# psaegert/bcnf

Measured on AMD Instinct MI355X. Metric: NLL-training samples/sec + log_prob max-abs-err vs ref, trajectory_FC_small, higher is better.
Workload: dtype f32; 1 GPU; trajectory_FC_small NLL training step (configs[1]); batch_per_gpu=4096, global_batch=4096, parallelism=dp1, hip_graph=True, n_blocks=32, n_conditions=80

## Files before the change

### bcnf_amd/csrc/bcnf_device.h

```cpp
#pragma once
#include <hip/hip_runtime.h>
#include <stdint.h>

#include <atomic>
#include <mutex>
#include <utility>

#include "../../include/bcnf_amd.h"

#define BCNF_WG 256
#define BCNF_ROWS 16
#define BCNF_TSTRIDE 17

typedef float floatx4 __attribute__((ext_vector_type(4)));

namespace bcnf_rt {
inline int hip_status(hipError_t e) { return e == hipSuccess ? 0 : BCNF_ERR_HIP_BASE + (int)e; }

constexpr size_t LDS_MAX = 160 * 1024;

struct Lds {
  size_t bytes, request;
  Lds(size_t b) : bytes(b), request(b) {}
  Lds(size_t b, size_t ceiling) : bytes(b), request(ceiling > b ? ceiling : b) {}
};

template <auto Kernel, typename... Args>
int launch(dim3 grid, dim3 block, Lds lds, hipStream_t stream, Args&&... args) {
  if (lds.bytes > LDS_MAX) return BCNF_ERR_UNSUPPORTED;
  if (lds.bytes > 0) {
    static std::atomic<size_t> granted{0};
    static std::mutex grow;
    if (lds.request > granted.load(std::memory_order_acquire)) {
      std::lock_guard<std::mutex> lk(grow);
      if (lds.request > granted.load(std::memory_order_relaxed)) {
        const hipError_t e = hipFuncSetAttribute(reinterpret_cast<const void*>(Kernel),
                                                 hipFuncAttributeMaxDynamicSharedMemorySize, (int)lds.request);
        if (e != hipSuccess) return hip_status(e);
        granted.store(lds.request, std::memory_order_release);
      }
    }
  }
  Kernel<<<grid, block, lds.bytes, stream>>>(std::forward<Args>(args)...);
  return hip_status(hipGetLastError());
}
}

constexpr int BCNF_GU = 8;
__device__ __forceinline__ void gather2_rows(const int64_t* __restrict__ idx, int n, int rpw,
                                             const float* __restrict__ s0, int c0, float* __restrict__ d0,
                                             const float* __restrict__ s1, int c1, float* __restrict__ d1,
                                             const long long* __restrict__ cursor, int bx) {
  if (cursor) idx += cursor[0] * n;
  const int r0 = bx * rpw, r1 = r0 + rpw < n ? r0 + rpw : n;
  const int cw = c0 + c1, total = (r1 - r0) * cw;
  for (int e0 = 0; e0 < total; e0 += BCNF_GU * BCNF_WG) {
    int r[BCNF_GU], col[BCNF_GU];
    long long src[BCNF_GU];
    float v[BCNF_GU];
#pragma unroll
    for (int u = 0; u < BCNF_GU; ++u) {
      int e = e0 + u * BCNF_WG + threadIdx.x;
      e = e < total ? e : total - 1;
      const int rr = e / cw;
      r[u] = r0 + rr;
      col[u] = e - rr * cw;
      src[u] = idx[r[u]];
    }
#pragma unroll
    for (int u = 0; u < BCNF_GU; ++u)
      v[u] = col[u] < c0 ? s0[src[u] * c0 + col[u]] : s1[src[u] * c1 + (col[u] - c0)];
#pragma unroll
    for (int u = 0; u < BCNF_GU; ++u) {
      if (e0 + u * BCNF_WG + (int)threadIdx.x >= total) continue;
      if (col[u] < c0)
        d0[r[u] * c0 + col[u]] = v[u];
      else
        d1[r[u] * c1 + (col[u] - c0)] = v[u];
    }
  }
}

struct BcnfGatherArgs {
  const int64_t* idx;
  const long long* cursor;
  const float* s0;
  float* d0;
  const float* s1;
  float* d1;
  int n, rpw, c0, c1, nwg;
};

inline void gather2_plan(long long n, int* rpw, int* nwg) {
  const int w = n < 512 ? (int)n : 512;
  *rpw = w > 0 ? (int)((n + w - 1) / w) : 1;
  *nwg = w > 0 ? (int)((n + *rpw - 1) / *rpw) : 0;
}
// ... 326 lines not shown
```

### bcnf_amd/csrc/bcnf_stack_bwd.hip

```cpp
#include "bcnf_stack_internal.h"
#include "bcnf_stack_rec.h"

namespace {
using namespace bcnf_small;
using bcnf_rt::launch;

#if BCNF_STAMPS
__device__ unsigned long long g_phase[32];
#endif

template <int NH>
struct BwdJobs {
  static constexpr int ND = NH + 6, NA = NH + 1;
  static constexpr int NW = NH + 2, NS = NH + 6;
  static constexpr int SUM_OFF = NW * 256;
  static constexpr int BLK = NW * 256 + NS * 16;
  __device__ static constexpr int wb(int c) { return c < NH ? c : NH; }
};

template <int NH>
__device__ __forceinline__ void bwd_grad_jobs(const float* __restrict__ Td, const float* __restrict__ Ta,
                                              float* __restrict__ out, int hw) {
  using J = BwdJobs<NH>;
  const int l64 = threadIdx.x & 63, q = l64 >> 4, r = l64 & 15;
  constexpr int UW = (J::NW + 3) / 4, US = (J::NS + 3) / 4;
  floatx4 a[UW], bv[UW], v[US];
  const int o = 4 * tile_slot(r, q);
#pragma unroll
  for (int u = 0; u < UW; ++u) {
    const int c = hw + 4 * u < J::NW ? hw + 4 * u : J::NW - 1;
    a[u] = *reinterpret_cast<const floatx4*>(Td + c * TILE + o);
    bv[u] = *reinterpret_cast<const floatx4*>(Ta + J::wb(c) * TILE + o);
  }
#pragma unroll
  for (int u = 0; u < US; ++u) {
    const int c = hw + 4 * u < J::NS ? hw + 4 * u : J::NS - 1;
    v[u] = *reinterpret_cast<const floatx4*>(Td + c * TILE + o);
  }
  floatx4 acc[UW];
#pragma unroll
  for (int u = 0; u < UW; ++u) acc[u] = floatx4{0.f, 0.f, 0.f, 0.f};
#pragma unroll
  for (int t = 0; t < 4; ++t)
#pragma unroll
    for (int u = 0; u < UW; ++u) acc[u] = mfma4(a[u][t], bv[u][t], acc[u]);
#pragma unroll
  for (int u = 0; u < US; ++u) {
    const float tot = sum_rows4((v[u][0] + v[u][1]) + (v[u][2] + v[u][3]));
    if (hw + 4 * u < J::NS && q == 0) out[J::SUM_OFF + 16 * (hw + 4 * u) + r] = tot;
  }
#pragma unroll
  for (int u = 0; u < UW; ++u)
    if (hw + 4 * u < J::NW) st4_wt_mfma(reinterpret_cast<floatx4*>(out + 256 * (hw + 4 * u)) + l64, acc[u]);
}

constexpr int BWD_WG = 2 * BCNF_WG;
constexpr int BWD_G4 = 3;

template <int NH>
__global__ __launch_bounds__(BWD_WG) void k_backward(BcnfLayout L, const float* __restrict__ pk,
                                                     const float* __restrict__ dz, const float* __restrict__ dldj,
                                                     const float* __restrict__ dloss, int nll, long long B,
                                                     const float* __restrict__ arec,
                                                     float* __restrict__ dy, float* __restrict__ d1,
                                                     float* __restrict__ slab_all, long long slab_stride,
                                                     const float* __restrict__ nll_part, float* __restrict__ loss_out,
                                                     uint64_t* rng_w, int32_t* guard) {
  static_assert(NH + 3 <= 4 * BWD_G4, "derivative slot");
  extern __shared__ __attribute__((aligned(16))) float smem[];
  using AR = ActRec<NH>;
  using RBk = RecB<NH>;
  using J = BwdJobs<NH>;
  const int RBL = 16 * L.RB;
  float* recB = smem;
  float* dT = recB + 2 * RING;
  float* aT = dT + 2 * J::ND * TILE;
  floatx4* gsl = reinterpret_cast<floatx4*>(aT + 3 * J::NA * TILE);
  const int nb = L.nb;
  const float* pbk = pk + L.pb_off;
  const bool helper = threadIdx.x >= BCNF_WG;
  const int t8 = (int)threadIdx.x & (BCNF_WG - 1);
  const int j = t8 & 15, s = sample_of(t8);
  const int tix = tile_ix(s, j);
  unsigned long long ph_t = BCNF_STAMPS ? __builtin_amdgcn_s_memtime() : 0ULL, ph_acc[4] = {0, 0, 0, 0};
#define PHS(i)                                                                                   \
  if (BCNF_STAMPS) {                                                                             \
    const unsigned long long _t = __builtin_amdgcn_s_memtime();                                  \
    ph_acc[i] += _t - ph_t;                                                                      \
    ph_t = _t;                                                                                   \
  }

  if (helper) {
    const int hw = __builtin_amdgcn_readfirstlane(t8 >> 6);
    float* slab = slab_all + (long long)blockIdx.x * slab_stride;
    const floatx4* arl = reinterpret_cast<const floatx4*>(arec) + (long long)blockIdx.x * AR::AR4 * BCNF_WG + t8;
    const long long ars = (long long)gridDim.x * AR::AR4 * BCNF_WG;
    struct Prep {
      Stage<STAGE_REC> sr;
      floatx4 rec[AR::AR4];
      float rec1[AR::AR1 > 0 ? AR::AR1 : 1];
      float sa, ba;
    };
    const float* ar1l = arec + ar1_off(nb, gridDim.x, AR::AR4) + (long long)blockIdx.x * AR::AR1 * BCNF_WG + t8;
    const long long ar1s = (long long)gridDim.x * AR::AR1 * BCNF_WG;
    auto prep_load = [&](Prep& P, int k) {
      P.sr.load_t(pbk + (long long)k * RBL, RBL, t8);
#pragma unroll
      for (int i = 0; i < AR::AR4; ++i) P.rec[i] = arl[(long long)k * ars + i * BCNF_WG];
#pragma unroll
      for (int i = 0; i < AR::AR1; ++i) P.rec1[i] = ar1l[(long long)k * ar1s + i * BCNF_WG];
      const float* an = pbk + (long long)k * RBL + j * L.RB + RBk::AN;
      P.sa = an[0];
      P.ba = an[1];
    };
    auto prep_store = [&](Prep& P, int k) {
#pragma unroll
      for (int i = 0; i < AR::AR4; ++i) asm volatile("" : "+v"(P.rec[i]));
#pragma unroll
      for (int i = 0; i < AR::AR1; ++i) asm volatile("" : "+v"(P.rec1[i]));
      asm volatile("" : "+v"(P.sa), "+v"(P.ba));
      float ar[4 * AR::AR4 + AR::AR1];
#pragma unroll
      for (int i = 0; i < AR::AR4; ++i) {
        ar[4 * i] = P.rec[i][0];
        ar[4 * i + 1] = P.rec[i][1];
        ar[4 * i + 2] = P.rec[i][2];
        ar[4 * i + 3] = P.rec[i][3];
      }
#pragma unroll
      for (int i = 0; i < AR::AR1; ++i) ar[4 * AR::AR4 + i] = P.rec1[i];
      float* ta = aT + (k % 3) * J::NA * TILE + tix;
#pragma unroll
      for (int l = 1; l <= NH; ++l) ta[l * TILE] = ar[AR::act(l - 1)];
      ta[0] = fmaf(P.sa, ar[AR::YA], P.ba);
      float gs[4 * BWD_G4];
#pragma unroll
      for (int l = 0; l < NH; ++l) gs[l] = ar[AR::gd(l)];
      gs[NH] = ar[AR::S];
      gs[NH + 1] = ar[AR::YA];
      gs[NH + 2] = ar[AR::YB];
#pragma unroll
      for (int i = NH + 3; i < 4 * BWD_G4; ++i) gs[i] = 0.f;
      floatx4* gd = gsl + (k & 1) * BWD_G4 * BCNF_WG + t8;
#pragma unroll
      for (int i = 0; i < BWD_G4; ++i) gd[i * BCNF_WG] = floatx4{gs[4 * i], gs[4 * i + 1], gs[4 * i + 2], gs[4 * i + 3]};
      P.sr.store_t(recB + (k & 1) * RING, t8);
    };
    Prep Pa, Pb;
    prep_load(Pa, nb - 1);
    prep_load(Pb, nb >= 2 ? nb - 2 : 0);
    prep_store(Pa, nb - 1);
    __syncthreads();
    auto step = [&](int k, Prep& Pc, Prep& Pnext) {
      PHS(0)
      prep_load(Pnext, k >= 2 ? k - 2 : 0);
      PHS(1)
      if (k + 1 < nb)
        bwd_grad_jobs<NH>(dT + ((k + 1) & 1) * J::ND * TILE, aT + ((k + 1) % 3) * J::NA * TILE,
                          slab + (long long)(k + 1) * J::BLK, hw);
      PHS(2)
      if (k >= 1) prep_store(Pc, k - 1);
      PHS(3)
      __syncthreads();
    };
    for (int k = nb - 1; k >= 0; k -= 2) {
      step(k, Pb, Pa);
      if (k == 0) break;
      step(k - 1, Pa, Pb);
    }
    bwd_grad_jobs<NH>(dT, aT, slab, hw);
  } else {
    const int tid = t8;
    const long long b = (long long)blockIdx.x * 16 + s;
    const bool valid = b < B;
    const long long bc = valid ? b : B - 1;
    const int D = L.D, Da = L.Da, Db = L.Db;
    float* d1l = d1 + bc * 16 + j;
    float* d1_dummy = d1 + (long long)nb * B * 16 + j;
    const long long hps = B * 16;

    float gya = 0.f, gyb = 0.f, dl = 0.f;
    if (valid) {
      if (nll) {
        const float sc = (dloss ? dloss[0] + dloss[1] : 1.f) / (float)B;
        gya = (j < Da) ? dz[b * D + j] * sc : 0.f;
        gyb = (j < Db) ? dz[b * D + Da + j] * sc : 0.f;
        dl = -sc;
      } else {
        if (dz) {
          gya = (j < Da) ? dz[b * D + j] : 0.f;
          gyb = (j < Db) ? dz[b * D + Da + j] : 0.f;
        }
        if (dldj) dl = dldj[b];
      }
    }
    __syncthreads();
    PHS(0)
    for (int k = nb - 1; k >= 0; --k) {
      const int cur = k & 1;
      float gs[4 * BWD_G4];
      {
        const floatx4* gd4 = gsl + cur * BWD_G4 * BCNF_WG + tid;
#pragma unroll
        for (int i = 0; i < BWD_G4; ++i) {
          const floatx4 v = gd4[i * BCNF_WG];
          gs[4 * i] = v[0];
          gs[4 * i + 1] = v[1];
          gs[4 * i + 2] = v[2];
          gs[4 * i + 3] = v[3];
        }
      }
      float* Tt = dT + cur * J::ND * TILE + tix;
      const float* R = recB + cur * RING + j * L.RB;
      float rb[RBk::USED];
      ld_rec<0, RBk::HID>(rb, R);
      __builtin_amdgcn_sched_barrier(0);
      const float* gd = gs;
      const float S = gs[NH], ya = gs[NH + 1], yb = gs[NH + 2];
      const float an_sa = rb[RBk::AN], an_sb = rb[RBk::AN + 2], an_bb = rb[RBk::AN + 3];
      const float xb = fmaf(an_sb, yb, an_bb);
      const float e = exp_fast(S);
      float gza, gzb;
      if (QBC_DEV(L, QBC_MIX)) mix_bc(rb + RBk::QT, gya, gyb, gza, gzb);
      else mix(rb + RBk::QT, gya, gyb, gza, gzb);
      ld16(rb + RBk::HID, R + RBk::HID);
      __builtin_amdgcn_sched_barrier(0);
      const float dT_ = gzb;
      const float dS = (j < Db) ? fmaf(gzb * e, xb, dl) : 0.f;
      const float dSp = dS * (1.f - S * S);
      const float dxb = gzb * e;
      Tt[NH * TILE] = dT_;
      Tt[(NH + 1) * TILE] = dSp;
      float da = 0.f, da2 = 0.f;
      if (QBC_DEV(L, QBC_HEAD)) bc9x2(dT_, rb + RBk::TT, da, dSp, rb + RBk::ST, da2);
      else rot16x2(dT_, rb + RBk::TT, da, dSp, rb + RBk::ST, da2);
      da += da2;
#pragma unroll
      for (int l = NH; l >= 2; --l) {
        ld16(rb + RBk::HID + 16 * (NH - l + 1), R + RBk::HID + 16 * (NH - l + 1));
        __builtin_amdgcn_sched_barrier(0);
        const float dpre = da * gd[l - 1];
        Tt[(l - 1) * TILE] = dpre;
        da = rot16(dpre, rb + RBk::HID + 16 * (NH - l), 0.f);
      }
      const float dpre1 = da * gd[0];
      Tt[0] = dpre1;
      *(valid ? d1l + k * hps : d1_dummy) = dpre1;
      const float dxa = rot16(dpre1, rb + RBk::W1T, gza);
      {
        const float inv_a = (j < Da) ? __builtin_amdgcn_rcpf(an_sa) : 0.f;
        const float inv_b = (j < Db) ? __builtin_amdgcn_rcpf(an_sb) : 0.f;
        Tt[(NH + 2) * TILE] = fmaf(dxa, ya, dl * inv_a);
        Tt[(NH + 3) * TILE] = dxa;
        Tt[(NH + 4) * TILE] = fmaf(dxb, yb, dl * inv_b);
        Tt[(NH + 5) * TILE] = dxb;
      }
      gya = an_sa * dxa;
      gyb = an_sb * dxb;
      PHS(1)
      __syncthreads();
      PHS(2)
    }
    if (dy && valid) {
      if (j < Da) dy[b * D + j] = gya;
      if (j < Db) dy[b * D + Da + j] = gyb;
    }
  }
#if BCNF_STAMPS
  if (blockIdx.x == 0 && (threadIdx.x == 0 || threadIdx.x == BCNF_WG))
    for (int i = 0; i < 4; ++i) g_phase[(helper ? 4 : 0) + i] = ph_acc[i];
#endif
#undef PHS
  if (loss_out && blockIdx.x == 0) {
    __syncthreads();
    nll_finalize<BWD_WG>(nll_part, (int)gridDim.x, B, loss_out, rng_w, guard, dT);
  }
}

}

namespace bcnf_small {

int launch_backward(const BcnfLayout& L, const float* pk, const float* dz, const float* dldj, const float* dloss,
                    int nll, long long B, const float* arec, float* dy, float* d1, float* slab, const float* part,
                    float* loss_out, uint64_t* rng_w, int32_t* guard, hipStream_t st) {
  return dispatch_nh(L.NH, [&](auto nh) -> int {
    constexpr int NH = decltype(nh)::value;
    if (!layout_matches<NH>(L)) return BCNF_ERR_ARG;
    const dim3 grid((unsigned)((B + 15) / 16));
    return launch<k_backward<NH>>(grid, dim3(BWD_WG), bwd_lds_bytes(L), st, L, pk, dz, dldj, dloss, nll, B, arec, dy,
                                  d1, slab, slab_stride_of(L), part, loss_out, rng_w, guard);
  });
}

#if BCNF_STAMPS
int bwd_debug_phases(unsigned long long* out) {
  return bcnf_rt::hip_status(hipMemcpyFromSymbol(out, HIP_SYMBOL(g_phase), sizeof(g_phase)));
}
#endif

}
```

### bcnf_amd/csrc/bcnf_stack_fwd.hip

```cpp
#include "bcnf_stack_internal.h"
#include "bcnf_stack_rec.h"

namespace {
using namespace bcnf_small;
using bcnf_rt::launch;

#if BCNF_STAMPS
__device__ unsigned long long g_phase[32];
#endif

struct ProjArgs {
  const float* h;
  const float* w1c;
  const float* b1c;
  long long ldh;
  int C, Cp, NKp;
};
struct RawArgs : RawForward {};
constexpr int RAW_WQ = 8;
constexpr int RAW_SIDE_Q = 4;
__host__ __device__ constexpr int raw_hs_pitch(int C) { return 16 * ((C + 15) / 16) + 4; }
__device__ __forceinline__ long long raw_row(const RawArgs& R, long long B, long long b) {
  return R.idx ? (long long)R.idx[(R.cursor ? R.cursor[0] * B : 0) + b] : b;
}

constexpr int HP_SMAX = 16;
constexpr int FWD_SLOTS = 3;
constexpr int FWD_HP = FWD_SLOTS * 4 * 256;
constexpr int FWD_HEAD = 24;

template <int NH, bool DROP, bool SAVE, bool RAW = false>
__global__ __launch_bounds__(2 * BCNF_WG) void k_forward(BcnfLayout L, const float* __restrict__ pk,
                                                    const float* __restrict__ y, ProjArgs P,
                                                    long long B, float* __restrict__ z, float* __restrict__ ldj_out,
                                                    float* __restrict__ logp, const uint64_t* rng,
                                                    float* __restrict__ arec, float* __restrict__ nll_part,
                                                    RawArgs R) {
  extern __shared__ __attribute__((aligned(16))) float smem[];
  const int RFL = 16 * L.RF;
  float* rec = smem;
  float* hpb = rec + FWD_SLOTS * RING;
  floatx4* mkb = reinterpret_cast<floatx4*>(hpb + FWD_HP);
  float* lps = hpb + FWD_HP + FWD_SLOTS * 8 * 256;
  float* hs = lps + 4;
  using AR = ActRec<NH>;
  static_assert(NH <= 8, "two float4 of dropout multipliers");
  const int nb = L.nb;
  const float* pf = pk + L.pf_off;
  const bool helper = threadIdx.x >= BCNF_WG;
  const int t8 = (int)threadIdx.x & (BCNF_WG - 1);
  const int j = t8 & 15, s = sample_of(t8);
  const long long b = (long long)blockIdx.x * 16 + s;
  const long long bc = b < B ? b : B - 1;
  uint64_t seed = 0, off = 0;
  if (DROP) { seed = rng[0]; off = rng[1]; }
  unsigned long long ph_t = BCNF_STAMPS ? __builtin_amdgcn_s_memtime() : 0ULL, ph_acc[3] = {0, 0, 0};
  const unsigned long long ph_t0 = ph_t;
  const unsigned long long ph_r0 = BCNF_STAMPS ? __builtin_amdgcn_s_memrealtime() : 0ULL;
  unsigned long long ph_b[2] = {0, 0};
#define PHB(i)                                                 \
  if (BCNF_STAMPS) ph_b[i] = __builtin_amdgcn_s_memtime() - ph_t0;
  unsigned long long ph_p[4] = {0, 0, 0, 0};
#define PHP(i)                                                                           \
  if (BCNF_STAMPS) {                                                                     \
    asm volatile("s_waitcnt vmcnt(0) lgkmcnt(0)" ::: "memory");                          \
    ph_p[i] = __builtin_amdgcn_s_memtime() - ph_t0;                                      \
  }
#define PHF(i)                                                                                   \
  if (BCNF_STAMPS) {                                                                             \
    const unsigned long long _t = __builtin_amdgcn_s_memtime();                                  \
    ph_acc[i] += _t - ph_t;                                                                      \
    ph_t = _t;                                                                                   \
  }

  if (helper) {
    const int hw = __builtin_amdgcn_readfirstlane(t8 >> 6);
    const int l64 = t8 & 63, lr = l64 & 15, lq = l64 >> 4;
    if constexpr (RAW) {
      const int Da = L.Da, C = L.C, X = R.X, H1 = L.H[1], D = L.D, an = L.an_size;
      const int nt = (C + 15) >> 4;
      const long long row = (long long)blockIdx.x * 16 + lr;
      const float* xrow = R.xpool + raw_row(R, B, row < B ? row : B - 1) * R.ldx;
      uint32_t tw[RAW_NSP];
#pragma unroll
      for (int i = 0; i < RAW_NSP / 4; ++i) {
        const uint4 v = reinterpret_cast<const uint4*>(R.table + t8 * RAW_NSP)[i];
        tw[4 * i] = v.x;
        tw[4 * i + 1] = v.y;
        tw[4 * i + 2] = v.z;
        tw[4 * i + 3] = v.w;
      }
      const int rb16 = 16 * L.RB, ch = (rb16 + BCNF_WG - 1) / BCNF_WG, n_units = nb * ch + L.NKp;
      const uint32_t* tpb = R.table + RAW_NSP * BCNF_WG;
      uint32_t pbe[RAW_SIDE_Q];
#pragma unroll
      for (int q = 0; q < RAW_SIDE_Q; ++q) {
        const int u = blockIdx.x + q * gridDim.x, n = (u % ch) * BCNF_WG + t8;
        pbe[q] = tpb[n < rb16 ? n : 0];
      }
      asm volatile("" ::: "memory");
      uint32_t srcb[RAW_NP + RAW_NQ], dstb[RAW_NP + RAW_NQ];
#pragma unroll
      for (int i = 0; i < RAW_NP + RAW_NQ; ++i) {
        srcb[i] = (tw[i] >> 12) * 4u;
        dstb[i] = (tw[i] & 4095u) * 4u;
      }
      uint32_t zw[RAW_NZ];
#pragma unroll
      for (int i = 0; i < RAW_NZ; ++i) zw[i] = tw[RAW_NP + RAW_NQ + i] & 4095u;
      PHP(0)
      int wo[RAW_TPW];
      uint32_t wok = 0;
#pragma unroll
      for (int i = 0; i < RAW_TPW; ++i) {
// ... 269 lines not shown
        for (int u = 0; u < RAW_WQ; ++u) {
          const int i = tid + u * BCNF_WG, c = i / XQ, q = i - c * XQ;
          if (i < nq) {
            floatx4 o;
#pragma unroll
            for (int r = 0; r < 4; ++r) o[r] = 4 * q + r < X ? __uint_as_float(v[u][r]) : 0.f;
            *reinterpret_cast<floatx4*>(ws + c * RAW_KP + 4 * q) = o;
          }
        }
        for (int i = nq > RAW_WQ * BCNF_WG ? tid + RAW_WQ * BCNF_WG : nq; i < nq; i += BCNF_WG) {
          const int c = i / XQ, q = i - c * XQ;
          const auto w = __builtin_amdgcn_raw_buffer_load_b128(rW, (c * X + 4 * q) * 4, 0, 0);
          floatx4 o;
#pragma unroll
          for (int r = 0; r < 4; ++r) o[r] = 4 * q + r < X ? __uint_as_float(w[r]) : 0.f;
          *reinterpret_cast<floatx4*>(ws + c * RAW_KP + 4 * q) = o;
        }
#pragma unroll
        for (int u = 0; u < NXQ; ++u) {
          const int i = tid + u * BCNF_WG;
          if (i < 16 * (RAW_KP / 4)) {
            const int rr = i / (RAW_KP / 4), q = i - rr * (RAW_KP / 4);
            *reinterpret_cast<floatx4*>(xs + rr * RAW_KP + 4 * q) = xo[u];
            const long long bb = (long long)blockIdx.x * 16 + rr;
            if (R.xdst && bb < B && 4 * q < X) {
              float* xd = R.xdst + bb * R.ldx + 4 * q;
              if (4 * q + 3 < X) {
                __builtin_memcpy(xd, &xo[u], sizeof(floatx4));
              } else {
#pragma unroll
                for (int r = 0; r < 4; ++r)
                  if (4 * q + r < X) xd[r] = xo[u][r];
              }
            }
          }
        }
      }
      PHP(0)
      __syncthreads();
      floatx4 acc[RAW_TPW][2];
#pragma unroll
      for (int i = 0; i < RAW_TPW; ++i) acc[i][0] = acc[i][1] = floatx4{0.f, 0.f, 0.f, 0.f};
#pragma unroll
      for (int u = 0; u < RAW_KP / 16; ++u) {
        if (16 * u >= X) break;
        const floatx4 xv = *reinterpret_cast<const floatx4*>(xs + lr * RAW_KP + 16 * u + 4 * lq);
#pragma unroll
        for (int i = 0; i < RAW_TPW; ++i) {
          const int ct = cw + 4 * i;
          if (16 * ct < C) {
            const int c = 16 * ct + lr;
            const floatx4 wv = *reinterpret_cast<const floatx4*>(ws + (c < C ? c : 0) * RAW_KP + 16 * u + 4 * lq);
#pragma unroll
            for (int r = 0; r < 4; ++r) acc[i][r & 1] = mfma4(wv[r], xv[r], acc[i][r & 1]);
          }
        }
      }
#pragma unroll
      for (int i = 0; i < RAW_TPW; ++i) {
        const int ct = cw + 4 * i;
        if (16 * ct < C) {
          floatx4 o;
#pragma unroll
          for (int r = 0; r < 4; ++r) {
            const int cc = 16 * ct + 4 * lq + r;
            o[r] = cc < C ? (acc[i][0][r] + acc[i][1][r]) + (R.bf ? hb[i][r] : 0.f) : 0.f;
          }
          *reinterpret_cast<floatx4*>(hs + lr * raw_hs_pitch(C) + 16 * ct + 4 * lq) = o;
        }
      }
      PHB(0)
      __syncthreads();
      PHB(1)
      if (R.ydst && b < B) {
        if (j < Da) R.ydst[b * D + j] = ya;
        if (j < Db) R.ydst[b * D + Da + j] = yb;
      }
    } else {
      ya = (j < Da) ? y[bc * D + j] : 0.f;
      yb = (j < Db) ? y[bc * D + Da + j] : 0.f;
      ldc = pk[L.ldc_off];
    }
    __syncthreads();
    float hd[FWD_HEAD], hq4[4];
    floatx4 mk0 = {1.f, 1.f, 1.f, 1.f}, mk1 = {1.f, 1.f, 1.f, 1.f};
    auto fetch_head = [&](int sl) {
      ld_rec<0, FWD_HEAD>(hd, rec + sl * RING + j * L.RF);
      const float* hq = hpb + sl * 1024 + 16 * s + j;
#pragma unroll
      for (int i = 0; i < 4; ++i) hq4[i] = hq[256 * i];
      if (DROP) {
        mk0 = mkb[(2 * sl) * BCNF_WG + tid];
        mk1 = mkb[(2 * sl + 1) * BCNF_WG + tid];
      }
    };
    fetch_head(0);
    float ldj = 0.f;
    int cur = 0;
    int gdim = gridDim.x;
    asm volatile("" : "+s"(gdim));
    floatx4* d4 = reinterpret_cast<floatx4*>(arec) + (long long)blockIdx.x * AR::AR4 * BCNF_WG + tid;
    float* d1p = arec + ar1_off(nb, gdim, AR::AR4) + (long long)blockIdx.x * AR::AR1 * BCNF_WG + tid;
    const long long d4s = (long long)gdim * AR::AR4 * BCNF_WG, d1s = (long long)gdim * AR::AR1 * BCNF_WG;
    for (int k = 0; k < nb; ++k) {
      const int nxt = cur == FWD_SLOTS - 1 ? 0 : cur + 1;
      float rr[RecF<NH>::USED];
#pragma unroll
      for (int i = 0; i < FWD_HEAD; ++i) rr[i] = hd[i];
      const float hpk = ((hq4[0] + hq4[1]) + hq4[2]) + hq4[3];
      const float msk[8] = {mk0[0], mk0[1], mk0[2], mk0[3], mk1[0], mk1[1], mk1[2], mk1[3]};
      const float xa = fmaf(rr[0], ya, rr[1]);
      const float xb = fmaf(rr[2], yb, rr[3]);
      float T, Sp;
      float ar[AR::AR];
      ar[AR::YA] = ya;
      ar[AR::YB] = yb;
      auto emit = [&](int q) {
        if (SAVE) st4_wt(d4 + q * BCNF_WG, floatx4{ar[4 * q], ar[4 * q + 1], ar[4 * q + 2], ar[4 * q + 3]});
      };
      mlp_forward_s<NH, SAVE, DROP>(rr, rec + cur * RING + j * L.RF, xa, hpk, msk, T, Sp, ar, emit, QBC_DEV(L, QBC_W1));
      const float Sv = tanh_bf(Sp);
      const float zb = fmaf(exp_fast(Sv), xb, T);
      ldj += Sv;
      if (SAVE) {
        ar[AR::S] = Sv;
#pragma unroll
        for (int q = 0; q < AR::AR4; ++q)
          if (AR::ready_layer(q) == NH + 1) emit(q);
#pragma unroll
        for (int i = 0; i < AR::AR1; ++i) st1_wt(d1p + i * BCNF_WG, ar[4 * AR::AR4 + i]);
        d4 += d4s;
        d1p += d1s;
      }
      fetch_head(nxt);
      if (QBC_DEV(L, QBC_MIX)) mix_bc(rr + RecF<NH>::Q, xa, zb, ya, yb);
      else mix(rr + RecF<NH>::Q, xa, zb, ya, yb);
      cur = nxt;
      PHF(1)
      asm volatile("s_barrier" ::: "memory");
      PHF(2)
    }
    if constexpr (RAW) ldc = ((lps[0] + lps[1]) + lps[2]) + lps[3];
    const float ltot = row_sum16(ldj) + ldc;
    const float q2 = row_sum16(ya * ya + yb * yb);
    if (j < Da) z[bc * D + j] = ya;
    if (j < Db) z[bc * D + Da + j] = yb;
    if (j == 0 && ldj_out) ldj_out[bc] = ltot;
    if (logp && j == 0) logp[bc] = -(0.5f * q2 - ltot) - 0.5f * (float)D * 1.8378770664093454836f;
    if (nll_part && j == 0) rec[s] = (b < B) ? 0.5f * q2 - ltot : 0.f;
  }
#if BCNF_STAMPS
  if (SAVE && blockIdx.x == 0 && (threadIdx.x == 0 || threadIdx.x == BCNF_WG))
  {
    for (int i = 0; i < 3; ++i) g_phase[8 + (helper ? 4 : 0) + i] = ph_acc[i];
    g_phase[helper ? 15 : 11] = (ph_b[1] << 32) | (ph_b[0] & 0xffffffffULL);
    for (int i = 0; i < 4; ++i) g_phase[16 + (helper ? 4 : 0) + i] = ph_p[i];
    g_phase[24 + (helper ? 2 : 0)] = __builtin_amdgcn_s_memtime() - ph_t0;
    g_phase[25 + (helper ? 2 : 0)] = __builtin_amdgcn_s_memrealtime() - ph_r0;
  }
#endif
#undef PHF
#undef PHB
#undef PHP
  if (nll_part) {
    __syncthreads();
    if (threadIdx.x == 0) {
      float acc = 0.f;
      for (int i = 0; i < 16; ++i) acc += rec[i];
      nll_part[blockIdx.x] = acc;
    }
  }
}

__global__ __launch_bounds__(BCNF_WG) void k_nll_finalize(const float* __restrict__ part, int nparts, long long B,
                                                          float* __restrict__ loss_out, uint64_t* rng_w,
                                                          int32_t* guard) {
  __shared__ float red[BCNF_WG];
  nll_finalize(part, nparts, B, loss_out, rng_w, guard, red);
}

}

namespace bcnf_small {

int launch_forward(const BcnfLayout& L, const float* pk, const float* y, const float* h, const float* fold, int X,
                   int ldx, long long B, float* z, float* ldj, float* logp, bool drop, const uint64_t* rng,
                   float* arec, float* part, const RawForward* raw, hipStream_t st) {
  const BcnfLayout Lp = fold ? fold_layout(L, X, ldx) : L;
  const float* pbase = fold ? fold : pk;
  const ProjArgs P{h, pbase + Lp.w1c_off, pbase + Lp.b1c_off, (long long)Lp.ldh, Lp.C, Lp.Cp, Lp.NKp};
  const dim3 grid((unsigned)((B + 15) / 16));
  const size_t lds = fwd2_lds_bytes(L, raw != nullptr);
  const bool save = arec != nullptr;
  const RawArgs R = raw ? RawArgs{*raw} : RawArgs{};
  return dispatch_nh(L.NH, [&](auto nh) -> int {
    constexpr int NH = decltype(nh)::value;
    if (!layout_matches<NH>(L)) return BCNF_ERR_ARG;
    if (P.Cp % 16 != 0 || P.Cp / 16 > HP_SMAX || P.C > P.Cp) return BCNF_ERR_UNSUPPORTED;
#define FWD(DR, SV, RW) \
  launch<k_forward<NH, DR, SV, RW>>(grid, dim3(2 * BCNF_WG), lds, st, L, pk, y, P, B, z, ldj, logp, rng, arec, part, R)
    if (raw) return !save ? BCNF_ERR_ARG : drop ? FWD(true, true, true) : FWD(false, true, true);
    if (save) return drop ? FWD(true, true, false) : FWD(false, true, false);
    return drop ? FWD(true, false, false) : FWD(false, false, false);
#undef FWD
  });
}

int launch_nll_finalize(const float* part, int nparts, long long B, float* loss_out, uint64_t* rng_w, int32_t* guard,
                        hipStream_t st) {
  return launch<k_nll_finalize>(dim3(1), dim3(BCNF_WG), 0, st, part, nparts, B, loss_out, rng_w, guard);
}

#if BCNF_STAMPS
int fwd_debug_phases(unsigned long long* out) {
  return bcnf_rt::hip_status(hipMemcpyFromSymbol(out, HIP_SYMBOL(g_phase), sizeof(g_phase)));
}
#endif

}
```

### bcnf_amd/csrc/bcnf_stack_rec.h

```cpp
#pragma once
#include "bcnf_stack_layout.h"

#ifdef BCNF_PHASE_STAMPS
#define BCNF_STAMPS 1
#else
#define BCNF_STAMPS 0
#endif
#define QBC_DEV(L, bit) (((L).qbc & (bit)) != 0)

#pragma GCC visibility push(hidden)
namespace bcnf_small {

template <int N>
struct Stage {
  floatx4 r[N];
  __device__ __forceinline__ void load(const float* __restrict__ g, int n) { load_t(g, n, (int)threadIdx.x); }
  __device__ __forceinline__ void store(float* __restrict__ s) const { store_t(s, (int)threadIdx.x); }
  __device__ __forceinline__ void load_t(const float* __restrict__ g, int n, int t) {
    const floatx4* g4 = reinterpret_cast<const floatx4*>(g);
    const int n4 = n >> 2;
#pragma unroll
    for (int i = 0; i < N; ++i) {
      const int idx = t + i * BCNF_WG;
      r[i] = g4[idx < n4 ? idx : 0];
    }
  }
  __device__ __forceinline__ void store_t(float* __restrict__ s, int t) const {
    floatx4* s4 = reinterpret_cast<floatx4*>(s);
#pragma unroll
    for (int i = 0; i < N; ++i) s4[t + i * BCNF_WG] = r[i];
  }
};

template <bool VEC>
__device__ __forceinline__ void load_rows64(const float* __restrict__ M, long long nrows, int ncols, long long ld,
                                            long long r0, int c0, floatx4* reg, int ones = -1) {
#pragma unroll
  for (int e = 0; e < 8; ++e) {
    const int i4 = threadIdx.x + 256 * e, row = i4 >> 5, col = c0 + (i4 & 31) * 4;
    const long long r = r0 + row < nrows ? r0 + row : nrows - 1;
    if (VEC) {
      const floatx4 v = *reinterpret_cast<const floatx4*>(M + r * ld + (col < ncols ? col : 0));
#pragma unroll
      for (int q = 0; q < 4; ++q) reg[e][q] = (r0 + row < nrows && col + q < ncols) ? v[q] : 0.f;
    } else {
#pragma unroll
      for (int q = 0; q < 4; ++q) {
        const int cq = col + q;
        const float v = M[r * ld + (cq < ncols ? cq : ncols - 1)];
        reg[e][q] = (r0 + row < nrows && cq < ncols) ? v : 0.f;
      }
    }
    if (ones >= 0) {
#pragma unroll
      for (int q = 0; q < 4; ++q)
        if (col + q == ones && r0 + row < nrows) reg[e][q] = 1.f;
    }
  }
}

template <int NH>
struct RecF {
  static constexpr int B1 = 4, W1 = 8, HID = 24, T = 24 + 17 * (NH - 1), S = T + 17;
  static constexpr int Q = (S + 17 + 3) & ~3, MLP_END = (S + 17 + 3) & ~3, USED = Q + 64;
};
template <int NH>
struct RecB {
  static constexpr int AN = 0, QT = 4, TT = 68, ST = 84, HID = 100, W1T = 100 + 16 * (NH - 1);
  static constexpr int USED = W1T + 16;
};
template <int NH>
struct ActRec {
  static constexpr int YA = 2 * NH, YB = 2 * NH + 1, S = 2 * NH + 2;
  static constexpr int AR = 2 * NH + 3, AR4 = AR / 4, AR1 = AR - 4 * AR4;
  __host__ __device__ static constexpr int act(int l) { return 2 * l; }
  __host__ __device__ static constexpr int gd(int l) { return 2 * l + 1; }
  __host__ __device__ static constexpr int ready_layer(int q) {
    int r = 0;
    for (int i = 4 * q; i < 4 * q + 4; ++i) {
      const int li = i < 2 * NH ? i / 2 + 1 : (i == S ? NH + 1 : 0);
      r = li > r ? li : r;
    }
    return r;
  }
};

template <int LO, int HI>
__device__ __forceinline__ void ld_rec(float* __restrict__ rr, const float* __restrict__ R) {
  static_assert(LO % 4 == 0 && HI % 4 == 0, "record slices are 16-B aligned");
  const floatx4* R4 = reinterpret_cast<const floatx4*>(R + LO);
#pragma unroll
  for (int i = 0; i < (HI - LO) / 4; ++i) {
    const floatx4 v = R4[i];
    rr[LO + 4 * i + 0] = v.x;
    rr[LO + 4 * i + 1] = v.y;
    rr[LO + 4 * i + 2] = v.z;
    rr[LO + 4 * i + 3] = v.w;
  }
}

template <int NH>
__device__ __forceinline__ void mlp_forward(const BcnfLayout& L, const float* __restrict__ rr, float x, float hp,
                                            uint32_t bits, float& T, float& Sp) {
  using F = RecF<NH>;
  float a = x;
#pragma unroll
  for (int l = 1; l <= NH; ++l) {
    const float* w = (l == 1) ? rr + F::W1 : rr + F::HID + 17 * (l - 2);
    const float bias = (l == 1) ? hp : w[16];
    const float pre = (l == 1 && QBC_DEV(L, QBC_W1)) ? bc10(a, w, bias) : rot16(a, w, bias);
    const float m = ((bits >> (l - 1)) & 1u) ? L.keep_scale : 0.f;
    a = gelu_f(pre) * m;
  }
  T = rr[F::T + 16];
  Sp = rr[F::S + 16];
  rot16x2(a, rr + F::T, T, a, rr + F::S, Sp);
}

constexpr int FWD_AHEAD = 2;
template <int NH>
__host__ __device__ constexpr int rf_stage_end(int l) {
  return l <= NH ? 24 + 17 * (l - 1) : (l == NH + 1 ? RecF<NH>::S + 17 : RecF<NH>::USED);
}
template <int NH>
__host__ __device__ constexpr int rf_stage_q(int l) {
  int q = 6;
  for (int i = 1; i <= l; ++i) {
    const int want = (rf_stage_end<NH>(i + FWD_AHEAD < NH + 2 ? i + FWD_AHEAD : NH + 2) + 3) / 4;
    q = i >= NH + 2 ? want : (want < q + 8 ? want : q + 8);
  }
  return q;
}
template <int NH>
__device__ __forceinline__ void rf_issue(float* __restrict__ rr, const float* __restrict__ R, int l) {
  const floatx4* R4 = reinterpret_cast<const floatx4*>(R);
#pragma unroll
  for (int q = rf_stage_q<NH>(l - 1); q < rf_stage_q<NH>(l); ++q) {
    const floatx4 v = R4[q];
    rr[4 * q] = v.x;
    rr[4 * q + 1] = v.y;
    rr[4 * q + 2] = v.z;
    rr[4 * q + 3] = v.w;
  }
  __builtin_amdgcn_sched_barrier(0);
}
template <int NH, bool KEEP, bool DROP, typename Emit>
__device__ __forceinline__ void mlp_forward_s(float* __restrict__ rr, const float* __restrict__ R, float x, float hp,
                                              const float* __restrict__ msk, float& T, float& Sp, float* ar,
                                              Emit&& emit, bool qbc) {
  static_assert(RecF<NH>::HID == 24, "stage 1 reads only the prefetched head (FWD_HEAD = 24)");
  using F = RecF<NH>;
  using AR = ActRec<NH>;
  float a = x;
#pragma unroll
  for (int l = 1; l <= NH; ++l) {
    rf_issue<NH>(rr, R, l);
    const float* w = (l == 1) ? rr + F::W1 : rr + F::HID + 17 * (l - 2);
    const float pre = (l == 1 && qbc) ? bc10(a, w, hp) : rot16(a, w, (l == 1) ? hp : w[16]);
    if (KEEP) {
      float g, dg;
      gelu_fg(pre, g, dg);
      a = DROP ? g * msk[l - 1] : g;
      ar[AR::act(l - 1)] = a;
      ar[AR::gd(l - 1)] = DROP ? dg * msk[l - 1] : dg;
#pragma unroll
      for (int q = 0; q < AR::AR4; ++q)
        if (AR::ready_layer(q) == l) emit(q);
    } else if (DROP) {
      float g, dg;
      gelu_fg(pre, g, dg);
      a = g * msk[l - 1];
    } else {
      a = gelu_f(pre);
    }
  }
  rf_issue<NH>(rr, R, NH + 1);
  T = rr[F::T + 16];
  Sp = rr[F::S + 16];
  rot16x2(a, rr + F::T, T, a, rr + F::S, Sp);
  rf_issue<NH>(rr, R, NH + 2);
}

__device__ __forceinline__ void mix(const float* __restrict__ rq, float a, float b, float& na, float& nbv) {
  na = 0.f;
  nbv = 0.f;
  rot16x2(a, rq, na, a, rq + 32, nbv);
  rot16x2(b, rq + 16, na, b, rq + 48, nbv);
}

template <int NTH = BCNF_WG>
static __device__ void nll_finalize(const float* __restrict__ part, int nparts, long long B, float* __restrict__ loss_out,
                             uint64_t* rng_w, int32_t* guard, float* __restrict__ red) {
  float acc = 0.f;
  for (int i = threadIdx.x; i < nparts; i += NTH) acc += part[i];
  red[threadIdx.x] = acc;
  __syncthreads();
  for (int w = NTH / 2; w > 0; w >>= 1) {
    if ((int)threadIdx.x < w) red[threadIdx.x] += red[threadIdx.x + w];
    __syncthreads();
  }
  if (threadIdx.x == 0) {
    const float nll = red[0] / (float)B;
    loss_out[0] = nll;
    loss_out[1] = nll;
    loss_out[2] = 0.f;
    bool halt = false;
    if (guard) {
      if (guard[BCNF_GUARD_DIVERGED]) {
        guard[BCNF_GUARD_HALTED] = 1;
        halt = true;
      } else if (guard[BCNF_GUARD_CHECK] && (nll > 1e5f || isnan(nll))) {
        guard[BCNF_GUARD_DIVERGED] = 1;
      }
    }
    if (rng_w && !halt) rng_w[1] += 1;
  }
}

__device__ __forceinline__ float sum_rows4(float v) {
  const auto p = __builtin_amdgcn_permlane32_swap(__float_as_uint(v), __float_as_uint(v), false, false);
  v = __uint_as_float(p[0]) + __uint_as_float(p[1]);
  const auto p2 = __builtin_amdgcn_permlane16_swap(__float_as_uint(v), __float_as_uint(v), false, false);
  return __uint_as_float(p2[0]) + __uint_as_float(p2[1]);
}

template <int NH>
constexpr int inv_m_rf() { return round_rec(RecF<NH>::USED); }
template <int NH>
bool layout_matches(const BcnfLayout& L) {
  return L.rf_b1 == RecF<NH>::B1 && L.rf_w1 == RecF<NH>::W1 && L.rf_hid == RecF<NH>::HID && L.rf_t == RecF<NH>::T &&
         L.rf_s == RecF<NH>::S && L.rf_q == RecF<NH>::Q && L.RF == inv_m_rf<NH>() &&
         L.PMB == (NH + 6) * 256 + (NH - 1) * 16 + 96 && L.rb_w1t == RecB<NH>::W1T &&
         L.rb_hid == RecB<NH>::HID && L.rb_tt == RecB<NH>::TT && L.rb_st == RecB<NH>::ST && L.rb_qt == RecB<NH>::QT &&
         L.rb_an == RecB<NH>::AN && L.RB >= RecB<NH>::USED;
}

}
#pragma GCC visibility pop
```

Measured before the change: 31.96 million samples/s.

## Specialize kernels on compressed-record layout and load only live record words

Makes the compressed (BC) record mode a compile-time template parameter of the forward and backward kernels, replacing runtime QBC flag checks. When BC is on, the forward kernel stops loading the dead tails of the head and mixing records. The backward kernel's helper waves stage only the live quads into LDS through a precomputed index map, so fewer global loads and LDS stores are issued per block. The cost is twice as many kernel instantiations. The layout check now rejects partial QBC flag combinations.

```diff
diff --git a/bcnf_amd/csrc/bcnf_device.h b/bcnf_amd/csrc/bcnf_device.h
--- a/bcnf_amd/csrc/bcnf_device.h
+++ b/bcnf_amd/csrc/bcnf_device.h
@@ -13,6 +13,7 @@
 #define BCNF_TSTRIDE 17
 
 typedef float floatx4 __attribute__((ext_vector_type(4)));
+typedef float floatx2 __attribute__((ext_vector_type(2)));
 
 namespace bcnf_rt {
 inline int hip_status(hipError_t e) { return e == hipSuccess ? 0 : BCNF_ERR_HIP_BASE + (int)e; }
diff --git a/bcnf_amd/csrc/bcnf_stack_bwd.hip b/bcnf_amd/csrc/bcnf_stack_bwd.hip
--- a/bcnf_amd/csrc/bcnf_stack_bwd.hip
+++ b/bcnf_amd/csrc/bcnf_stack_bwd.hip
@@ -57,7 +57,7 @@
 constexpr int BWD_WG = 2 * BCNF_WG;
 constexpr int BWD_G4 = 3;
 
-template <int NH>
+template <int NH, bool BC>
 __global__ __launch_bounds__(BWD_WG) void k_backward(BcnfLayout L, const float* __restrict__ pk,
                                                      const float* __restrict__ dz, const float* __restrict__ dldj,
                                                      const float* __restrict__ dloss, int nll, long long B,
@@ -95,8 +95,20 @@
     float* slab = slab_all + (long long)blockIdx.x * slab_stride;
     const floatx4* arl = reinterpret_cast<const floatx4*>(arec) + (long long)blockIdx.x * AR::AR4 * BCNF_WG + t8;
     const long long ars = (long long)gridDim.x * AR::AR4 * BCNF_WG;
+    constexpr int LQ = RBk::live_quads(BC), LSTAGE = (16 * LQ + BCNF_WG - 1) / BCNF_WG;
+    constexpr bool MAPPED = BC && LSTAGE < STAGE_REC;
+    constexpr int BSTAGE = MAPPED ? LSTAGE : STAGE_REC;
+    int six[BSTAGE];
+    if constexpr (MAPPED) {
+      const int rb4 = L.RB >> 2;
+#pragma unroll
+      for (int i = 0; i < BSTAGE; ++i) {
+        const int n = t8 + i * BCNF_WG, lane = n / LQ, c = n - lane * LQ;
+        six[i] = n < 16 * LQ ? lane * rb4 + RBk::live_quad(true, c) : RBk::dead_quad();
+      }
+    }
     struct Prep {
-      Stage<STAGE_REC> sr;
+      Stage<BSTAGE> sr;
       floatx4 rec[AR::AR4];
       float rec1[AR::AR1 > 0 ? AR::AR1 : 1];
       float sa, ba;
@@ -104,7 +116,8 @@
     const float* ar1l = arec + ar1_off(nb, gridDim.x, AR::AR4) + (long long)blockIdx.x * AR::AR1 * BCNF_WG + t8;
     const long long ar1s = (long long)gridDim.x * AR::AR1 * BCNF_WG;
     auto prep_load = [&](Prep& P, int k) {
-      P.sr.load_t(pbk + (long long)k * RBL, RBL, t8);
+      if constexpr (MAPPED) P.sr.load_ix(pbk + (long long)k * RBL, six);
+      else P.sr.load_t(pbk + (long long)k * RBL, RBL, t8);
 #pragma unroll
       for (int i = 0; i < AR::AR4; ++i) P.rec[i] = arl[(long long)k * ars + i * BCNF_WG];
 #pragma unroll
@@ -144,7 +157,8 @@
       floatx4* gd = gsl + (k & 1) * BWD_G4 * BCNF_WG + t8;
 #pragma unroll
       for (int i = 0; i < BWD_G4; ++i) gd[i * BCNF_WG] = floatx4{gs[4 * i], gs[4 * i + 1], gs[4 * i + 2], gs[4 * i + 3]};
-      P.sr.store_t(recB + (k & 1) * RING, t8);
+      if constexpr (MAPPED) P.sr.store_ix(recB + (k & 1) * RING, six);
+      else P.sr.store_t(recB + (k & 1) * RING, t8);
     };
     Prep Pa, Pb;
     prep_load(Pa, nb - 1);
@@ -213,7 +227,10 @@
       float* Tt = dT + cur * J::ND * TILE + tix;
       const float* R = recB + cur * RING + j * L.RB;
       float rb[RBk::USED];
-      ld_rec<0, RBk::HID>(rb, R);
+      ld_rec<0, RBk::qt_end(BC)>(rb, R);
+      __builtin_amdgcn_sched_barrier(0);
+      ld_rec<RBk::TT, RBk::TT + RBk::head_len(BC)>(rb, R);
+      ld_rec<RBk::ST, RBk::ST + RBk::head_len(BC)>(rb, R);
       __builtin_amdgcn_sched_barrier(0);
       const float* gd = gs;
       const float S = gs[NH], ya = gs[NH + 1], yb = gs[NH + 2];
@@ -221,7 +238,7 @@
       const float xb = fmaf(an_sb, yb, an_bb);
       const float e = exp_fast(S);
       float gza, gzb;
-      if (QBC_DEV(L, QBC_MIX)) mix_bc(rb + RBk::QT, gya, gyb, gza, gzb);
+      if constexpr (BC) mix_bc(rb + RBk::QT, gya, gyb, gza, gzb);
       else mix(rb + RBk::QT, gya, gyb, gza, gzb);
       ld16(rb + RBk::HID, R + RBk::HID);
       __builtin_amdgcn_sched_barrier(0);
@@ -232,7 +249,7 @@
       Tt[NH * TILE] = dT_;
       Tt[(NH + 1) * TILE] = dSp;
       float da = 0.f, da2 = 0.f;
-      if (QBC_DEV(L, QBC_HEAD)) bc9x2(dT_, rb + RBk::TT, da, dSp, rb + RBk::ST, da2);
+      if constexpr (BC) bc9x2(dT_, rb + RBk::TT, da, dSp, rb + RBk::ST, da2);
       else rot16x2(dT_, rb + RBk::TT, da, dSp, rb + RBk::ST, da2);
       da += da2;
 #pragma unroll
@@ -288,8 +305,11 @@
     constexpr int NH = decltype(nh)::value;
     if (!layout_matches<NH>(L)) return BCNF_ERR_ARG;
     const dim3 grid((unsigned)((B + 15) / 16));
-    return launch<k_backward<NH>>(grid, dim3(BWD_WG), bwd_lds_bytes(L), st, L, pk, dz, dldj, dloss, nll, B, arec, dy,
-                                  d1, slab, slab_stride_of(L), part, loss_out, rng_w, guard);
+#define BWD(BC) \
+  launch<k_backward<NH, BC>>(grid, dim3(BWD_WG), bwd_lds_bytes(L), st, L, pk, dz, dldj, dloss, nll, B, arec, dy, d1, \
+                             slab, slab_stride_of(L), part, loss_out, rng_w, guard)
+    return layout_bc(L) ? BWD(true) : BWD(false);
+#undef BWD
   });
 }
 
diff --git a/bcnf_amd/csrc/bcnf_stack_fwd.hip b/bcnf_amd/csrc/bcnf_stack_fwd.hip
--- a/bcnf_amd/csrc/bcnf_stack_fwd.hip
+++ b/bcnf_amd/csrc/bcnf_stack_fwd.hip
@@ -29,7 +29,7 @@
 constexpr int FWD_HP = FWD_SLOTS * 4 * 256;
 constexpr int FWD_HEAD = 24;
 
-template <int NH, bool DROP, bool SAVE, bool RAW = false>
+template <int NH, bool DROP, bool SAVE, bool RAW, bool BC>
 __global__ __launch_bounds__(2 * BCNF_WG) void k_forward(BcnfLayout L, const float* __restrict__ pk,
                                                     const float* __restrict__ y, ProjArgs P,
                                                     long long B, float* __restrict__ z, float* __restrict__ ldj_out,
@@ -465,10 +465,11 @@
       ldc = pk[L.ldc_off];
     }
     __syncthreads();
+    constexpr int HEAD_END = RecF<NH>::head_end(BC);
     float hd[FWD_HEAD], hq4[4];
     floatx4 mk0 = {1.f, 1.f, 1.f, 1.f}, mk1 = {1.f, 1.f, 1.f, 1.f};
     auto fetch_head = [&](int sl) {
-      ld_rec<0, FWD_HEAD>(hd, rec + sl * RING + j * L.RF);
+      ld_rec<0, HEAD_END>(hd, rec + sl * RING + j * L.RF);
       const float* hq = hpb + sl * 1024 + 16 * s + j;
 #pragma unroll
       for (int i = 0; i < 4; ++i) hq4[i] = hq[256 * i];
@@ -489,7 +490,7 @@
       const int nxt = cur == FWD_SLOTS - 1 ? 0 : cur + 1;
       float rr[RecF<NH>::USED];
 #pragma unroll
-      for (int i = 0; i < FWD_HEAD; ++i) rr[i] = hd[i];
+      for (int i = 0; i < HEAD_END; ++i) rr[i] = hd[i];
       const float hpk = ((hq4[0] + hq4[1]) + hq4[2]) + hq4[3];
       const float msk[8] = {mk0[0], mk0[1], mk0[2], mk0[3], mk1[0], mk1[1], mk1[2], mk1[3]};
       const float xa = fmaf(rr[0], ya, rr[1]);
@@ -501,7 +502,7 @@
       auto emit = [&](int q) {
         if (SAVE) st4_wt(d4 + q * BCNF_WG, floatx4{ar[4 * q], ar[4 * q + 1], ar[4 * q + 2], ar[4 * q + 3]});
       };
-      mlp_forward_s<NH, SAVE, DROP>(rr, rec + cur * RING + j * L.RF, xa, hpk, msk, T, Sp, ar, emit, QBC_DEV(L, QBC_W1));
+      mlp_forward_s<NH, SAVE, DROP, BC>(rr, rec + cur * RING + j * L.RF, xa, hpk, msk, T, Sp, ar, emit);
       const float Sv = tanh_bf(Sp);
       const float zb = fmaf(exp_fast(Sv), xb, T);
       ldj += Sv;
@@ -516,7 +517,7 @@
         d1p += d1s;
       }
       fetch_head(nxt);
-      if (QBC_DEV(L, QBC_MIX)) mix_bc(rr + RecF<NH>::Q, xa, zb, ya, yb);
+      if constexpr (BC) mix_bc(rr + RecF<NH>::Q, xa, zb, ya, yb);
       else mix(rr + RecF<NH>::Q, xa, zb, ya, yb);
       cur = nxt;
       PHF(1)
@@ -580,12 +581,14 @@
     constexpr int NH = decltype(nh)::value;
     if (!layout_matches<NH>(L)) return BCNF_ERR_ARG;
     if (P.Cp % 16 != 0 || P.Cp / 16 > HP_SMAX || P.C > P.Cp) return BCNF_ERR_UNSUPPORTED;
-#define FWD(DR, SV, RW) \
-  launch<k_forward<NH, DR, SV, RW>>(grid, dim3(2 * BCNF_WG), lds, st, L, pk, y, P, B, z, ldj, logp, rng, arec, part, R)
+#define FWD1(DR, SV, RW, BC) \
+  launch<k_forward<NH, DR, SV, RW, BC>>(grid, dim3(2 * BCNF_WG), lds, st, L, pk, y, P, B, z, ldj, logp, rng, arec, part, R)
+#define FWD(DR, SV, RW) (layout_bc(L) ? FWD1(DR, SV, RW, true) : FWD1(DR, SV, RW, false))
     if (raw) return !save ? BCNF_ERR_ARG : drop ? FWD(true, true, true) : FWD(false, true, true);
     if (save) return drop ? FWD(true, true, false) : FWD(false, true, false);
     return drop ? FWD(true, false, false) : FWD(false, false, false);
 #undef FWD
+#undef FWD1
   });
 }
 
diff --git a/bcnf_amd/csrc/bcnf_stack_rec.h b/bcnf_amd/csrc/bcnf_stack_rec.h
--- a/bcnf_amd/csrc/bcnf_stack_rec.h
+++ b/bcnf_amd/csrc/bcnf_stack_rec.h
@@ -30,6 +30,16 @@
 #pragma unroll
     for (int i = 0; i < N; ++i) s4[t + i * BCNF_WG] = r[i];
   }
+  __device__ __forceinline__ void load_ix(const float* __restrict__ g, const int* ix) {
+    const floatx4* g4 = reinterpret_cast<const floatx4*>(g);
+#pragma unroll
+    for (int i = 0; i < N; ++i) r[i] = g4[ix[i]];
+  }
+  __device__ __forceinline__ void store_ix(float* __restrict__ s, const int* ix) const {
+    floatx4* s4 = reinterpret_cast<floatx4*>(s);
+#pragma unroll
+    for (int i = 0; i < N; ++i) s4[ix[i]] = r[i];
+  }
 };
 
 template <bool VEC>
@@ -59,15 +69,31 @@
   }
 }
 
+constexpr int BC_W1 = 10, BC_Q = 38, BC_HEAD = 9;
+__host__ __device__ constexpr int quads(int n) { return (n + 3) / 4; }
 template <int NH>
 struct RecF {
   static constexpr int B1 = 4, W1 = 8, HID = 24, T = 24 + 17 * (NH - 1), S = T + 17;
   static constexpr int Q = (S + 17 + 3) & ~3, MLP_END = (S + 17 + 3) & ~3, USED = Q + 64;
+  __host__ __device__ static constexpr int head_end(bool bc) { return bc ? W1 + BC_W1 : HID; }
+  __host__ __device__ static constexpr int live_end(bool bc) { return bc ? Q + BC_Q : USED; }
 };
 template <int NH>
 struct RecB {
   static constexpr int AN = 0, QT = 4, TT = 68, ST = 84, HID = 100, W1T = 100 + 16 * (NH - 1);
   static constexpr int USED = W1T + 16;
+  __host__ __device__ static constexpr int qt_end(bool bc) { return bc ? QT + BC_Q : TT; }
+  __host__ __device__ static constexpr int head_len(bool bc) { return bc ? BC_HEAD : 16; }
+  __host__ __device__ static constexpr int live_quads(bool bc) {
+    return bc ? quads(qt_end(true)) + 2 * quads(BC_HEAD) + (USED - HID) / 4 : USED / 4;
+  }
+  __host__ __device__ static constexpr int live_quad(bool bc, int c) {
+    if (!bc) return c;
+    const int nq = quads(qt_end(true)), nh = quads(BC_HEAD);
+    return c < nq ? c : c < nq + nh ? TT / 4 + (c - nq) : c < nq + 2 * nh ? ST / 4 + (c - nq - nh)
+                                                                        : HID / 4 + (c - nq - 2 * nh);
+  }
+  __host__ __device__ static constexpr int dead_quad() { return quads(qt_end(true)); }
 };
 template <int NH>
 struct ActRec {
@@ -85,9 +111,19 @@
   }
 };
 
+template <int N>
+__device__ __forceinline__ void ld_rec_tail(float* __restrict__ rr, const float* __restrict__ R, int e) {
+  static_assert(N >= 0 && N < 4, "less than a quad");
+  if (N >= 2) {
+    const floatx2 v = *reinterpret_cast<const floatx2*>(R + e);
+    rr[e] = v.x;
+    rr[e + 1] = v.y;
+  }
+  if (N & 1) rr[e + (N & 2)] = R[e + (N & 2)];
+}
 template <int LO, int HI>
 __device__ __forceinline__ void ld_rec(float* __restrict__ rr, const float* __restrict__ R) {
-  static_assert(LO % 4 == 0 && HI % 4 == 0, "record slices are 16-B aligned");
+  static_assert(LO % 4 == 0 && HI >= LO, "record slices start 16-B aligned");
   const floatx4* R4 = reinterpret_cast<const floatx4*>(R + LO);
 #pragma unroll
   for (int i = 0; i < (HI - LO) / 4; ++i) {
@@ -97,6 +133,7 @@
     rr[LO + 4 * i + 2] = v.z;
     rr[LO + 4 * i + 3] = v.w;
   }
+  ld_rec_tail<(HI - LO) % 4>(rr, R, LO + (HI - LO) / 4 * 4);
 }
 
 template <int NH>
@@ -118,24 +155,28 @@
 }
 
 constexpr int FWD_AHEAD = 2;
-template <int NH>
+template <int NH, bool BC>
 __host__ __device__ constexpr int rf_stage_end(int l) {
-  return l <= NH ? 24 + 17 * (l - 1) : (l == NH + 1 ? RecF<NH>::S + 17 : RecF<NH>::USED);
-}
-template <int NH>
+  return l <= NH ? 24 + 17 * (l - 1) : (l == NH + 1 ? RecF<NH>::S + 17 : RecF<NH>::live_end(BC));
+}
+template <int NH, bool BC>
 __host__ __device__ constexpr int rf_stage_q(int l) {
   int q = 6;
   for (int i = 1; i <= l; ++i) {
-    const int want = (rf_stage_end<NH>(i + FWD_AHEAD < NH + 2 ? i + FWD_AHEAD : NH + 2) + 3) / 4;
+    const int want = (rf_stage_end<NH, BC>(i + FWD_AHEAD < NH + 2 ? i + FWD_AHEAD : NH + 2) + 3) / 4;
     q = i >= NH + 2 ? want : (want < q + 8 ? want : q + 8);
   }
   return q;
 }
-template <int NH>
+template <int NH, bool BC>
 __device__ __forceinline__ void rf_issue(float* __restrict__ rr, const float* __restrict__ R, int l) {
   const floatx4* R4 = reinterpret_cast<const floatx4*>(R);
 #pragma unroll
-  for (int q = rf_stage_q<NH>(l - 1); q < rf_stage_q<NH>(l); ++q) {
+  for (int q = rf_stage_q<NH, BC>(l - 1); q < rf_stage_q<NH, BC>(l); ++q) {
+    if (4 * q + 4 > RecF<NH>::live_end(BC)) {
+      ld_rec_tail<RecF<NH>::live_end(BC) % 4>(rr, R, 4 * q);
+      continue;
+    }
     const floatx4 v = R4[q];
     rr[4 * q] = v.x;
     rr[4 * q + 1] = v.y;
@@ -144,19 +185,19 @@
   }
   __builtin_amdgcn_sched_barrier(0);
 }
-template <int NH, bool KEEP, bool DROP, typename Emit>
+template <int NH, bool KEEP, bool DROP, bool BC, typename Emit>
 __device__ __forceinline__ void mlp_forward_s(float* __restrict__ rr, const float* __restrict__ R, float x, float hp,
                                               const float* __restrict__ msk, float& T, float& Sp, float* ar,
-                                              Emit&& emit, bool qbc) {
+                                              Emit&& emit) {
   static_assert(RecF<NH>::HID == 24, "stage 1 reads only the prefetched head (FWD_HEAD = 24)");
   using F = RecF<NH>;
   using AR = ActRec<NH>;
   float a = x;
 #pragma unroll
   for (int l = 1; l <= NH; ++l) {
-    rf_issue<NH>(rr, R, l);
+    rf_issue<NH, BC>(rr, R, l);
     const float* w = (l == 1) ? rr + F::W1 : rr + F::HID + 17 * (l - 2);
-    const float pre = (l == 1 && qbc) ? bc10(a, w, hp) : rot16(a, w, (l == 1) ? hp : w[16]);
+    const float pre = (l == 1 && BC) ? bc10(a, w, hp) : rot16(a, w, (l == 1) ? hp : w[16]);
     if (KEEP) {
       float g, dg;
       gelu_fg(pre, g, dg);
@@ -174,11 +215,11 @@
       a = gelu_f(pre);
     }
   }
-  rf_issue<NH>(rr, R, NH + 1);
+  rf_issue<NH, BC>(rr, R, NH + 1);
   T = rr[F::T + 16];
   Sp = rr[F::S + 16];
   rot16x2(a, rr + F::T, T, a, rr + F::S, Sp);
-  rf_issue<NH>(rr, R, NH + 2);
+  rf_issue<NH, BC>(rr, R, NH + 2);
 }
 
 __device__ __forceinline__ void mix(const float* __restrict__ rq, float a, float b, float& na, float& nbv) {
@@ -232,8 +273,9 @@
          L.rf_s == RecF<NH>::S && L.rf_q == RecF<NH>::Q && L.RF == inv_m_rf<NH>() &&
          L.PMB == (NH + 6) * 256 + (NH - 1) * 16 + 96 && L.rb_w1t == RecB<NH>::W1T &&
          L.rb_hid == RecB<NH>::HID && L.rb_tt == RecB<NH>::TT && L.rb_st == RecB<NH>::ST && L.rb_qt == RecB<NH>::QT &&
-         L.rb_an == RecB<NH>::AN && L.RB >= RecB<NH>::USED;
-}
+         L.rb_an == RecB<NH>::AN && L.RB >= RecB<NH>::USED && (L.qbc == 0 || L.qbc == (QBC_W1 | QBC_MIX | QBC_HEAD));
+}
+inline bool layout_bc(const BcnfLayout& L) { return L.qbc == (QBC_W1 | QBC_MIX | QBC_HEAD); }
 
 }
 #pragma GCC visibility pop
```

Measured after the change: 32.73 million samples/s (median of 6 runs). 1.02x the previous value.
